# jacobswan1/ViTCAP

Hardware: AMD Instinct MI355X
Metric: images/sec end-to-end greedy caption (20 tok), ViT-B/16-384 (higher is better)
Workload: dtype bf16; 1 GPU; BASELINE configs[1]: ViT-B/16-384 greedy decode (20 tok), batch 64 bf16 per GPU, seeded random-init weights, uniform(-1,1) 384x384 images resident in HBM; batch_per_gpu=64, global_batch=64, decode=greedy, max_length=20, parallelism=replicas x1 (no data-path collective), launch=2-slot batch pipeline (encode of step i+1 || decode of step i), eager launches, streams_per_gpu=2

## Files before the change

### vitcap_amd/csrc/gemm.hip

```cpp
#include <stdio.h>
#include <stdlib.h>

#include "common.h"
#include "gemm_args.h"


#include <algorithm>
#include <mutex>
#include <utility>
#include <vector>

namespace {

int tile_group_n(int tiles_n) {
  return tiles_n > 9 ? 3 : tiles_n;
}

}
int vc_tile_group_n(int tiles_n) { return tile_group_n(tiles_n); }
namespace {

__device__ __forceinline__ void glds16(const void* g, void* lds) {
  __builtin_amdgcn_global_load_lds((const __attribute__((address_space(1))) void*)g,
                                   (__attribute__((address_space(3))) void*)lds, 16, 0, 0);
// ... 215 lines not shown
      const u32x2_t t = __builtin_amdgcn_permlane32_swap(r[c][k], r[c + 2][k], false, false);
      r[c][k] = t[0];
      r[c + 2][k] = t[1];
    }
#pragma unroll
  for (int c = 0; c < 4; c += 2)
#pragma unroll
    for (int k = 0; k < NREG; ++k) {
      const u32x2_t t = __builtin_amdgcn_permlane16_swap(r[c][k], r[c + 1][k], false, false);
      r[c][k] = t[0];
      r[c + 1][k] = t[1];
    }
}

template <int ACT, int OUT_F32, bool HAS_RES, int NI>
__device__ __forceinline__ void epilogue_direct(f32x4 (&acc)[NI][4], const GemmArgs& p, int row0, int col0, int lane) {
  const int frow = lane & 15, fk = lane >> 4;
  f32x4 bias4[4];
#pragma unroll
  for (int j = 0; j < 4; ++j) {
    const int n = col0 + j * 16 + fk * 4;
    bias4[j] = (p.bias && n < p.N) ? *(const f32x4*)(p.bias + n) : f32x4{0.f, 0.f, 0.f, 0.f};
  }
  const int ncol = col0 + fk * 16;
  const bool col_ok = ncol < p.N;
  f32x4 rres[2][4];
#define ISSUE_RES_D(i_)                                                                                    \
  if (HAS_RES) {                                                                                           \
    const int m_ = row0 + (i_) * 16 + frow;                                                                \
    _Pragma("unroll") for (int q = 0; q < 4; ++q)                                                          \
      rres[(i_) & 1][q] = (m_ < p.M && col_ok) ? *(const f32x4*)(p.res + (size_t)m_ * p.ldr + ncol + q * 4) \
                                               : f32x4{0.f, 0.f, 0.f, 0.f};                                \
  }
  ISSUE_RES_D(0);
#pragma unroll
  for (int i = 0; i < NI; ++i) {
    if (i + 1 < NI) { ISSUE_RES_D(i + 1); }
    const int m = row0 + i * 16 + frow;
    f32x4 v[4];
#pragma unroll
    for (int j = 0; j < 4; ++j) {
      v[j] = acc[i][j] + bias4[j];
      if (ACT == VITCAP_ACT_GELU_ERF) {
        v[j] = gelu_erf4(v[j]);
      }
    }
    if (OUT_F32) {
      unsigned r[4][4];
#pragma unroll
      for (int j = 0; j < 4; ++j)
#pragma unroll
        for (int e = 0; e < 4; ++e) r[j][e] = __float_as_uint(v[j][e]);
      lane_tile_transpose<4>(r);
      if (m < p.M && col_ok) {
        float* dst = (float*)p.C + (size_t)m * p.ldc + ncol;
#pragma unroll
        for (int q = 0; q < 4; ++q) {
          f32x4 o = f32x4{__uint_as_float(r[q][0]), __uint_as_float(r[q][1]), __uint_as_float(r[q][2]), __uint_as_float(r[q][3])};
          if (HAS_RES) o += rres[i & 1][q];
          *(f32x4*)(dst + q * 4) = o;
        }
      }
    } else {
      unsigned r[4][2];
#pragma unroll
      for (int j = 0; j < 4; ++j) {
        r[j][0] = pack2bf(v[j][0], v[j][1]);
        r[j][1] = pack2bf(v[j][2], v[j][3]);
      }
      lane_tile_transpose<2>(r);
      if (m < p.M && col_ok) {
        bf16_t* dst = (bf16_t*)p.C + (size_t)m * p.ldc + ncol;
        uint4 o0, o1;
        o0.x = r[0][0]; o0.y = r[0][1]; o0.z = r[1][0]; o0.w = r[1][1];
        o1.x = r[2][0]; o1.y = r[2][1]; o1.z = r[3][0]; o1.w = r[3][1];
        *(uint4*)dst = o0;
        *(uint4*)(dst + 8) = o1;
      }
    }
  }
#undef ISSUE_RES_D
}

template <int ACT, int OUT_F32, bool HAS_RES, int PH, int MT>
__device__ __forceinline__ void gemm256_tile(const GemmArgs& p, char* smem, const int m0, const int n0, const int cidx = 0) {
  constexpr int BK = 64;
  constexpr int A_BYTES = 256 * BK * 2, BUF_BYTES = 2 * A_BYTES;
  constexpr int WR = 32 * MT;
  constexpr int NI = 2 * MT;
  constexpr int NP = MT + 4;
  constexpr bool EXTRAS = (PH & 8) != 0;
  constexpr bool LN = (PH & 512) != 0;

  const int tid = threadIdx.x;
  const int lane = tid & 63;
  const int w = __builtin_amdgcn_readfirstlane(tid >> 6);
  const int grp = w >> 2;
  const int wm = w >> 2, wn = w & 3;

  const int srow = lane >> 3;
  const int schunk = (lane & 7) ^ (srow & 7);
  const bf16_t* aptr[MT];
  const bf16_t* wptr[4];
#pragma unroll
  for (int i = 0; i < MT; ++i) {
    int r = m0 + w * (8 * MT) + i * 8 + srow;
    r = r < p.M ? r : p.M - 1;
    aptr[i] = p.A + (size_t)r * p.lda + schunk * 8;
  }
#pragma unroll
  for (int i = 0; i < 4; ++i) {
    int c = n0 + w * 32 + i * 8 + srow;
    c = c < p.N ? c : p.N - 1;
    wptr[i] = p.W + (size_t)c * p.ldw + schunk * 8;
  }
#define STAGE_PIECES(q0_, q1_, buf_, k0_)                                                                          \
  _Pragma("unroll") for (int q = (q0_); q < (q1_); ++q) {                                                          \
    if (q < MT)                                                                                                    \
      glds16(aptr[q < MT ? q : 0] + (k0_), smem + (buf_) * BUF_BYTES + (w * (8 * MT) + q * 8) * 128);              \
    else                                                                                                           \
      glds16(wptr[q < MT ? 0 : q - MT] + (k0_), smem + (buf_) * BUF_BYTES + A_BYTES + (w * 32 + (q - MT) * 8) * 128); \
  }
#define STAGE_SLOT(s_, buf_, k0_) STAGE_PIECES(2 * (s_), (2 * (s_) + 2 < NP ? 2 * (s_) + 2 : NP), buf_, k0_)

  f32x4 acc[NI][4];
#pragma unroll
  for (int i = 0; i < NI; ++i)
#pragma unroll
    for (int j = 0; j < 4; ++j) acc[i][j] = f32x4{0.f, 0.f, 0.f, 0.f};

  const int frow = lane & 15;
  const int fk = lane >> 4;
  const int coff0 = ((0 * 4 + fk) ^ (frow & 7)) * 16;
  const int coff1 = ((1 * 4 + fk) ^ (frow & 7)) * 16;
  const int a_base = (wm * WR + frow) * 128;
  const int b_base = A_BYTES + (wn * 64 + frow) * 128;
  const int nk = p.K / BK;

  bf16x8 afr[MT][2];
  bf16x8 bfr[2][2][2];

#define LOAD_A(buf_, mh_)                                                                        \
  _Pragma("unroll") for (int mt = 0; mt < MT; ++mt) {                                            \
    const char* ra_ = smem + (buf_) * BUF_BYTES + a_base + ((mh_) * MT + mt) * 16 * 128;         \
    afr[mt][0] = *(const bf16x8*)(ra_ + coff0);                                                  \
    afr[mt][1] = *(const bf16x8*)(ra_ + coff1);                                                  \
  }
#define LOAD_B(buf_, nh_)                                                                        \
  _Pragma("unroll") for (int nt = 0; nt < 2; ++nt) {                                             \
    const char* rb_ = smem + (buf_) * BUF_BYTES + b_base + ((nh_) * 2 + nt) * 16 * 128;          \
    bfr[nh_][nt][0] = *(const bf16x8*)(rb_ + coff0);                                             \
    bfr[nh_][nt][1] = *(const bf16x8*)(rb_ + coff1);                                             \
  }
#define END_LOAD()                                          \
  asm volatile("s_waitcnt lgkmcnt(0)" ::: "memory");        \
  __builtin_amdgcn_sched_barrier(0);                        \
  __builtin_amdgcn_s_barrier()
#define COMPUTE(mh_, nh_)                                                                               \
  __builtin_amdgcn_s_setprio(1);                                                                        \
  _Pragma("unroll") for (int ks = 0; ks < 2; ++ks)                                                      \
    _Pragma("unroll") for (int mt = 0; mt < MT; ++mt)                                                   \
      _Pragma("unroll") for (int nt = 0; nt < 2; ++nt)                                                  \
        acc[(mh_) * MT + mt][(nh_) * 2 + nt] = __builtin_amdgcn_mfma_f32_16x16x32_bf16(                 \
            bfr[nh_][nt][ks], afr[mt][ks], acc[(mh_) * MT + mt][(nh_) * 2 + nt], 0, 0, 0);              \
  __builtin_amdgcn_s_setprio(0)

  STAGE_PIECES(0, NP, 0, 0);
  if (nk > 1) {
    STAGE_SLOT(0, 1, BK);
    asm volatile("s_waitcnt vmcnt(2)" ::: "memory");
  } else {
    asm volatile("s_waitcnt vmcnt(0)" ::: "memory");
  }
  __builtin_amdgcn_s_barrier();
  if (grp == 1) __builtin_amdgcn_s_barrier();

  for (int t = 0; t < nk; ++t) {
    const int buf = t & 1;
    const bool more = t + 1 < nk;
    const bool more2 = t + 2 < nk;
    LOAD_A(buf, 0);
    LOAD_B(buf, 0);
    if (more) { STAGE_SLOT(1, buf ^ 1, (t + 1) * BK); }
    END_LOAD();
    COMPUTE(0, 0);
    __builtin_amdgcn_s_barrier();
    LOAD_B(buf, 1);
    if (more) { STAGE_SLOT(2, buf ^ 1, (t + 1) * BK); }
    END_LOAD();
    COMPUTE(0, 1);
    __builtin_amdgcn_s_barrier();
    LOAD_A(buf, 1);
    if (more) { STAGE_SLOT(3, buf ^ 1, (t + 1) * BK); }
    END_LOAD();
    COMPUTE(1, 1);
    __builtin_amdgcn_s_barrier();
    if (more2) { STAGE_SLOT(0, buf, (t + 2) * BK); }
    if (grp == 1) {
      if (more2) asm volatile("s_waitcnt vmcnt(2)" ::: "memory");
      else asm volatile("s_waitcnt vmcnt(0)" ::: "memory");
    }
    __builtin_amdgcn_s_barrier();
    COMPUTE(1, 0);
    if (grp == 0) {
      if (more2) asm volatile("s_waitcnt vmcnt(2)" ::: "memory");
      else asm volatile("s_waitcnt vmcnt(0)" ::: "memory");
    }
    __builtin_amdgcn_s_barrier();
  }
  if (grp == 0) __builtin_amdgcn_s_barrier();
#undef STAGE_PIECES
#undef STAGE_SLOT
#undef LOAD_A
#undef LOAD_B
#undef END_LOAD
#undef COMPUTE

  constexpr int EP_ROWB = 272;
  char* ep = smem + w * (64 * EP_ROWB);
  const int er = lane >> 4, ec = (lane & 15) * 4;
  const int ncol = n0 + wn * 64 + ec;
  f32x4 bias4 = f32x4{0.f, 0.f, 0.f, 0.f};
  if (p.bias && ncol < p.N) bias4 = *(const f32x4*)(p.bias + ncol);
  const bool col_ok = ncol < p.N;
  f32x4 rres[2][2 * MT];
#define ROWS_OF(m_, orow_, rrow_)                                             \
  int orow_ = (m_), rrow_ = (m_);                                             \
  if (p.row_group > 0) {                                                      \
    const int g_ = (m_) / p.row_group, in_ = (m_) - g_ * p.row_group;         \
    orow_ = g_ * p.out_group_rows + p.out_row_off + in_;                      \
    rrow_ = p.res_periodic ? in_ : orow_;                                     \
  }
#define ISSUE_RES(c_)                                                                                        \
  if (HAS_RES) {                                                                                             \
    _Pragma("unroll") for (int it = 0; it < 2 * MT; ++it) {                                                  \
      const int m_ = m0 + wm * WR + (c_) * (8 * MT) + it * 4 + er;                                           \
      ROWS_OF(m_, o_, r_);                                                                                   \
      (void)o_;                                                                                              \
      rres[(c_) & 1][it] = (m_ < p.M && col_ok) ? *(const f32x4*)(p.res + (size_t)r_ * p.ldr + ncol)        \
                                                : f32x4{0.f, 0.f, 0.f, 0.f};                                 \
    }                                                                                                        \
  }
  if (ACT == VITCAP_ACT_GELU_ERF && !OUT_F32 && !HAS_RES && !(EXTRAS && p.zout) && !(EXTRAS && p.aux) && p.row_group == 0 &&
      (p.N & 15) == 0 && (p.ldc & 7) == 0) {
    epilogue_direct<ACT, OUT_F32, HAS_RES, NI>(acc, p, m0 + wm * WR, n0 + wn * 64, lane);
    return;
  }
  if constexpr (!OUT_F32 && !HAS_RES) {
    if (p.row_group == 0 && (p.N & 7) == 0 && (p.ldc & 7) == 0 && (!(EXTRAS && p.zout) || (p.ldz & 7) == 0) && (!(EXTRAS && p.aux) || (p.ldaux & 7) == 0)) {
      const int wr = lane >> 3, wc = (lane & 7) * 8;
      const int ncw = n0 + wn * 64 + wc;
      const bool okc = ncw < p.N;
      f32x4 b_lo = f32x4{0.f, 0.f, 0.f, 0.f}, b_hi = b_lo;
      f32x4 cs_lo = f32x4{0.f, 0.f, 0.f, 0.f}, cs_hi = cs_lo;
      if (p.bias && ncw < p.N) {
        b_lo = *(const f32x4*)(p.bias + ncw);
        b_hi = *(const f32x4*)(p.bias + ncw + 4);
      }
#pragma unroll
      for (int hm = 0; hm < 2; ++hm) {
        uint4 axv[2 * MT];
        if (EXTRAS && p.aux) {
#pragma unroll
          for (int it = 0; it < 2 * MT; ++it) {
            const int m = m0 + wm * WR + hm * (16 * MT) + it * 8 + wr;
            axv[it] = (m < p.M && okc) ? *(const uint4*)(p.aux + (size_t)m * p.ldaux + ncw) : uint4{0u, 0u, 0u, 0u};
          }
        }
#pragma unroll
        for (int i = 0; i < MT; ++i)
#pragma unroll
          for (int j = 0; j < 4; ++j)
            *(f32x4*)(ep + (i * 16 + frow) * EP_ROWB + (j * 16 + fk * 4) * 4) = acc[hm * MT + i][j];
#pragma unroll
        for (int it = 0; it < 2 * MT; ++it) {
          const int rl = it * 8 + wr;
          f32x4 v0 = *(const f32x4*)(ep + rl * EP_ROWB + wc * 4);
          f32x4 v1 = *(const f32x4*)(ep + rl * EP_ROWB + wc * 4 + 16);
          const int m = m0 + wm * WR + hm * (16 * MT) + rl;
          const bool ok = m < p.M && okc;
          v0 += b_lo;
          v1 += b_hi;
          if (EXTRAS && p.aux) {
            const uint4 a = axv[it];
            v0 *= f32x4{__uint_as_float(a.x << 16), __uint_as_float(a.x & 0xffff0000u), __uint_as_float(a.y << 16),
                        __uint_as_float(a.y & 0xffff0000u)};
            v1 *= f32x4{__uint_as_float(a.z << 16), __uint_as_float(a.z & 0xffff0000u), __uint_as_float(a.w << 16),
                        __uint_as_float(a.w & 0xffff0000u)};
          }
          if (ACT == VITCAP_ACT_GELU_ERF) {
            if (EXTRAS && p.zout) {
              f32x4 d0, d1;
              v0 = gelu_erf4_grad(v0, d0);
              v1 = gelu_erf4_grad(v1, d1);
              if (ok) {
                uint4 zo;
                zo.x = pack2bf(d0[0], d0[1]);
                zo.y = pack2bf(d0[2], d0[3]);
                zo.z = pack2bf(d1[0], d1[1]);
                zo.w = pack2bf(d1[2], d1[3]);
                *(uint4*)(p.zout + (size_t)m * p.ldz + ncw) = zo;
              }
            } else {
              v0 = gelu_erf4(v0);
              v1 = gelu_erf4(v1);
            }
          }
          if (ok) {
            uint4 o;
            o.x = pack2bf(v0[0], v0[1]);
            o.y = pack2bf(v0[2], v0[3]);
            o.z = pack2bf(v1[0], v1[1]);
            o.w = pack2bf(v1[2], v1[3]);
            *(uint4*)((bf16_t*)p.C + (size_t)m * p.ldc + ncw) = o;
            if (EXTRAS && p.colsum) {
              cs_lo += f32x4{__uint_as_float(o.x << 16), __uint_as_float(o.x & 0xffff0000u), __uint_as_float(o.y << 16),
                             __uint_as_float(o.y & 0xffff0000u)};
              cs_hi += f32x4{__uint_as_float(o.z << 16), __uint_as_float(o.z & 0xffff0000u), __uint_as_float(o.w << 16),
                             __uint_as_float(o.w & 0xffff0000u)};
            }
          }
        }
      }
      if (EXTRAS && p.colsum) {
#pragma unroll
        for (int e = 0; e < 4; ++e) {
#pragma unroll
          for (int o = 8; o <= 32; o <<= 1) {
            cs_lo[e] += __shfl_xor(cs_lo[e], o, 64);
            cs_hi[e] += __shfl_xor(cs_hi[e], o, 64);
          }
        }
        if (wr == 0 && okc) {
#pragma unroll
          for (int e = 0; e < 4; ++e) {
            atomicAdd(p.colsum + ncw + e, cs_lo[e]);
            atomicAdd(p.colsum + ncw + 4 + e, cs_hi[e]);
          }
        }
      }
      return;
    }
  }
  const __amdgpu_buffer_rsrc_t ln_rc = vc_rsrc(LN ? (const char*)p.C + (size_t)m0 * p.ldc * 4 : nullptr, LN ? (long long)(p.M - m0) * p.ldc * 4 : 0);
  ISSUE_RES(0);
#pragma unroll
  for (int hm = 0; hm < 2; ++hm) {
#pragma unroll
    for (int i = 0; i < MT; ++i)
#pragma unroll
      for (int j = 0; j < 4; ++j)
        *(f32x4*)(ep + (i * 16 + frow) * EP_ROWB + (j * 16 + fk * 4) * 4) = acc[hm * MT + i][j];
#pragma unroll
    for (int ch = 0; ch < 2; ++ch) {
      const int c = hm * 2 + ch;
      if (c + 1 < 4) { ISSUE_RES(c + 1); }
#pragma unroll
      for (int it = 0; it < 2 * MT; ++it) {
        const int rl = ch * (8 * MT) + it * 4 + er;
        f32x4 v = *(const f32x4*)(ep + rl * EP_ROWB + ec * 4);
        const int m = m0 + wm * WR + hm * (16 * MT) + rl;
        const bool ok = m < p.M && col_ok;
        ROWS_OF(m, orow, rrow);
        (void)rrow;
        v += bias4;
        if (EXTRAS && p.aux && ok) {
          const bf16x4 za = *(const bf16x4*)(p.aux + (size_t)orow * p.ldaux + ncol);
          v *= f32x4{(float)za[0], (float)za[1], (float)za[2], (float)za[3]};
        }
        if (ACT == VITCAP_ACT_GELU_ERF) {
          if (EXTRAS && p.zout) {
            f32x4 d;
            v = gelu_erf4_grad(v, d);
            if (ok) {
              uint2 zo;
              zo.x = pack2bf(d[0], d[1]);
              zo.y = pack2bf(d[2], d[3]);
              *(uint2*)(p.zout + (size_t)orow * p.ldz + ncol) = zo;
            }
          } else {
            v = gelu_erf4(v);
          }
        }
        if (HAS_RES) v += rres[c & 1][it];
        if (ok) {
          if (OUT_F32) {
            if constexpr (LN) {
              __builtin_amdgcn_raw_buffer_store_b128(__builtin_bit_cast(vc_u32x4, v), ln_rc, (unsigned)((orow - m0) * p.ldc + ncol) * 4u, 0, 16);
            } else {
              *(f32x4*)((float*)p.C + (size_t)orow * p.ldc + ncol) = v;
            }
          } else {
            uint2 o;
            o.x = pack2bf(v[0], v[1]);
            o.y = pack2bf(v[2], v[3]);
            *(uint2*)((bf16_t*)p.C + (size_t)orow * p.ldc + ncol) = o;
          }
        }
      }
    }
  }
#undef ISSUE_RES
#undef ROWS_OF
  if constexpr (LN) {
    asm volatile("s_waitcnt vmcnt(0)" ::: "memory");
    __syncthreads();
    int* s_flag = (int*)smem;
    if (tid == 0) {
      const int old = __hip_atomic_fetch_add(p.ln_cnt + cidx, 1, __ATOMIC_RELAXED, __HIP_MEMORY_SCOPE_AGENT);
      const int last = old == p.tiles_n - 1;
      if (last) __hip_atomic_store(p.ln_cnt + cidx, 0, __ATOMIC_RELAXED, __HIP_MEMORY_SCOPE_AGENT);
      *s_flag = last;
    }
    __syncthreads();
    if (*s_flag == 0) return;
    if (!p.ln_out && !p.ln_out_f) return;
    if (tid == 0) __builtin_amdgcn_fence(__ATOMIC_ACQUIRE, "agent");
    __syncthreads();
    const int rows = p.M - m0 < 64 * MT ? p.M - m0 : 64 * MT;
    constexpr int RB = 8;
    for (int r0 = w * RB; r0 < rows; r0 += 8 * RB) {
      f32x4 v[RB][3];
#pragma unroll
      for (int j = 0; j < RB; ++j)
#pragma unroll
        for (int i = 0; i < 3; ++i)
          v[j][i] = __builtin_bit_cast(f32x4, __builtin_amdgcn_raw_buffer_load_b128(ln_rc, (unsigned)((r0 + j) * p.ldc + i * 256 + lane * 4) * 4u, 0, 0));
#pragma unroll
      for (int j = 0; j < RB; ++j) {
        const int row = m0 + r0 + j;
        if (r0 + j < rows)
          ln_row(v[j], p.ln_g, p.ln_b, p.ln_eps, lane, p.ln_out ? p.ln_out + (size_t)row * D768 : nullptr,
                 p.ln_out_f ? p.ln_out_f + (size_t)row * D768 : nullptr);
      }
    }
  }
}

#ifndef VC_GEMM256_VGPRS
#define VC_GEMM256_VGPRS 224
#endif
template <int ACT, int OUT_F32, bool HAS_RES, int PH, int MTS>
__global__ __launch_bounds__(512) __attribute__((amdgpu_num_vgpr(VC_GEMM256_VGPRS))) void gemm_nt_256_kernel(GemmArgs p) {
  extern __shared__ __attribute__((aligned(16))) char smem[];
  int bid = blockIdx.x;
  const bool small = MTS != 0 && bid >= p.n_big;
  if (small) bid -= p.n_big;
  const int tiles_m = small ? p.tiles_m_small : p.tiles_m;
  {
    const int nwg = tiles_m * p.tiles_n;
    const int q = nwg >> 3, r = nwg & 7, xcd = bid & 7;
    bid = (xcd < r ? xcd * (q + 1) : r * (q + 1) + (xcd - r) * q) + (bid >> 3);
  }
  const int per_g = tiles_m * p.group_n;
  const int gi = bid / per_g, rem = bid - gi * per_g;
  const int gleft = p.tiles_n - gi * p.group_n;
  const int gw = gleft < p.group_n ? gleft : p.group_n;
  int tm = rem / gw;
  const int tn = gi * p.group_n + rem - tm * gw;
  if ((p.rev != 0) != ((gi & 1) != 0)) tm = tiles_m - 1 - tm;
  if (!small) {
    gemm256_tile<ACT, OUT_F32, HAS_RES, PH, 4>(p, smem, tm * 256, tn * 256, tm);
  } else {
    if constexpr (MTS != 0) gemm256_tile<ACT, OUT_F32, HAS_RES, PH, MTS>(p, smem, p.tiles_m * 256 + tm * (64 * MTS), tn * 256, p.tiles_m + tm);
  }
}

struct TilePlan { int tm_big, mts, tm_small; };
TilePlan plan_tiles(int M, int tiles_n, int K) {
  static const int n_cu = [] {
    int dev = 0;
    hipDeviceProp_t prop;
    if (hipGetDevice(&dev) == hipSuccess && hipGetDeviceProperties(&prop, dev) == hipSuccess && prop.multiProcessorCount > 0)
      return prop.multiProcessorCount;
    return 256;
  }();
  const int tm_full = (M + 255) / 256;
  TilePlan best{tm_full, 0, 0};
  struct Key { int M, tn, K; };
  static std::mutex mu;
  static std::vector<std::pair<Key, TilePlan>> cache;
  {
    std::lock_guard<std::mutex> g(mu);
    for (const auto& e : cache)
      if (e.first.M == M && e.first.tn == tiles_n && e.first.K == K) return e.second;
  }
  const float c3 = 0.80f, c2 = 0.60f;
  float best_t = ceilf((float)(tm_full * tiles_n) / n_cu);
  const float need = best_t * 0.97f;
  const int span = (int)(2.5f * n_cu / tiles_n) + 2;
  std::vector<float> heap;
  for (int mts = 3; mts >= 2; --mts) {
    const float cs = mts == 3 ? c3 : c2;
    for (int tb = tm_full - 1; tb >= 0 && tb >= tm_full - span; --tb) {
      const int rows_left = M - tb * 256;
      const int ts = (rows_left + 64 * mts - 1) / (64 * mts);
      const int nb = tb * tiles_n, ns = ts * tiles_n;
      heap.assign(n_cu, 0.f);
      for (int j = 0; j < n_cu; ++j) heap[j] = -(float)(nb / n_cu + (j < nb % n_cu ? 1 : 0));
      std::make_heap(heap.begin(), heap.end());
      float end = nb ? (float)((nb + n_cu - 1) / n_cu) : 0.f;
      for (int i = 0; i < ns; ++i) {
        std::pop_heap(heap.begin(), heap.end());
        const float f = -heap.back() + cs;
        heap.back() = -f;
        std::push_heap(heap.begin(), heap.end());
        end = f > end ? f : end;
      }
      if (end < need && end < best_t - 1e-4f) { best_t = end; best = TilePlan{tb, mts, ts}; }
    }
  }
  std::lock_guard<std::mutex> g(mu);
  cache.push_back({Key{M, tiles_n, K}, best});
  return best;
}

template <int ACT, int OUT_F32, bool HAS_RES, int PH, int MTS>
int launch_256_t(const GemmArgs& p, int nwg, hipStream_t s) {
  constexpr int smem = 8 * 64 * 272;
  auto kern = gemm_nt_256_kernel<ACT, OUT_F32, HAS_RES, PH, MTS>;
  VC_FUNC_SMEM(kern, smem);
  VC_LAUNCH_GEMM(kern, dim3(nwg), dim3(512), smem, s, p);
  VC_LAUNCH_CHECK("gemm_nt_256");
  return VITCAP_OK;
}

template <int ACT, int OUT_F32, bool HAS_RES, int PH>
int launch_256(const GemmArgs& a, hipStream_t s, int mix = 0) {
  if constexpr ((PH & 512) != 0) mix = 0;
  GemmArgs p = a;
  p.tiles_n = (a.N + 255) / 256;
  p.group_n = tile_group_n(p.tiles_n);
  TilePlan pl{(a.M + 255) / 256, 0, 0};
  if (a.aux || a.zout || a.colsum) mix = 0;
  if (mix < 0) pl = plan_tiles(a.M, p.tiles_n, a.K);
  else if (mix > 0) pl = TilePlan{0, mix, (a.M + 64 * mix - 1) / (64 * mix)};
  p.tiles_m = pl.tm_big;
  p.tiles_m_small = pl.tm_small;
  p.n_big = pl.tm_big * p.tiles_n;
  const int nwg = p.n_big + pl.tm_small * p.tiles_n;
  if constexpr ((PH & 512) == 0) {
    if (a.aux || a.zout || a.colsum) return launch_256_t<ACT, OUT_F32, HAS_RES, PH | 8, 0>(p, nwg, s);
    if (pl.mts == 3) return launch_256_t<ACT, OUT_F32, HAS_RES, PH, 3>(p, nwg, s);
    if (pl.mts == 2) return launch_256_t<ACT, OUT_F32, HAS_RES, PH, 2>(p, nwg, s);
  }
  return launch_256_t<ACT, OUT_F32, HAS_RES, PH, 0>(p, nwg, s);
}

template <int PH>
int dispatch_256(const GemmArgs& a, int act, int out_f32, hipStream_t s, int mix = 0) {
  const bool res = a.res != nullptr;
#define CASE(ACT_, OUT_)                                                  \
  if (act == ACT_ && out_f32 == OUT_)                                     \
    return res ? launch_256<ACT_, OUT_, true, PH>(a, s, mix) : launch_256<ACT_, OUT_, false, PH>(a, s, mix);
  CASE(VITCAP_ACT_NONE, 0)
  CASE(VITCAP_ACT_NONE, 1)
  CASE(VITCAP_ACT_GELU_ERF, 0)
  CASE(VITCAP_ACT_GELU_ERF, 1)
#undef CASE
  vitcap_set_error("gemm(256): unsupported act %d / out %d", act, out_f32);
  return VITCAP_EINVAL;
}


struct SkinnyArgs {
  GemmArgs g;
  int split_k;
  int kc;
  size_t slab;
};

template <int WAVES_M, int ACT, int OUT_F32, bool HAS_RES, bool PARTIAL>
__global__ __launch_bounds__(256) void gemm_skinny_kernel(SkinnyArgs q) {
  constexpr int WAVES_N = 4 / WAVES_M;
  constexpr int BM = 32 * WAVES_M, BN = 32 * WAVES_N;
  const GemmArgs& p = q.g;
  VC_LIVE_EXIT(p.live);
  const int lane = threadIdx.x & 63;
  const int w = __builtin_amdgcn_readfirstlane(threadIdx.x >> 6);
  const int wm = w / WAVES_N, wn = w % WAVES_N;
  const int n0 = blockIdx.x * BN + wn * 32;
  const int m0 = blockIdx.y * BM + wm * 32;
  const int kz = blockIdx.z;
  const int kbeg = kz * q.kc;
  const int frow = lane & 15, fk = lane >> 4;

  const bf16_t* ap[2];
  const bf16_t* wp[2];
#pragma unroll
  for (int i = 0; i < 2; ++i) {
    int r = m0 + i * 16 + frow;
    r = r < p.M ? r : p.M - 1;
    ap[i] = p.A + (size_t)r * p.lda + kbeg + fk * 8;
    int c = n0 + i * 16 + frow;
    c = c < p.N ? c : p.N - 1;
    wp[i] = p.W + (size_t)c * p.ldw + kbeg + fk * 8;
  }
  f32x4 acc[2][2];
#pragma unroll
  for (int i = 0; i < 2; ++i)
#pragma unroll
    for (int j = 0; j < 2; ++j) acc[i][j] = f32x4{0.f, 0.f, 0.f, 0.f};

  bf16x8 a0[4][2], w0[4][2], a1[4][2], w1[4][2];
#define LOADSET(A_, W_, k0_)                                                   \
  _Pragma("unroll") for (int s_ = 0; s_ < 4; ++s_) {                           \
    _Pragma("unroll") for (int i_ = 0; i_ < 2; ++i_) {                         \
      A_[s_][i_] = *(const bf16x8*)(ap[i_] + (k0_) + s_ * 32);                 \
      W_[s_][i_] = *(const bf16x8*)(wp[i_] + (k0_) + s_ * 32);                 \
    }                                                                          \
  }
#define MMASET(A_, W_)                                                                          \
  _Pragma("unroll") for (int s_ = 0; s_ < 4; ++s_)                                              \
    _Pragma("unroll") for (int i_ = 0; i_ < 2; ++i_)                                            \
      _Pragma("unroll") for (int j_ = 0; j_ < 2; ++j_)                                          \
        acc[i_][j_] = __builtin_amdgcn_mfma_f32_16x16x32_bf16(W_[s_][j_], A_[s_][i_], acc[i_][j_], 0, 0, 0);

  const int nch = q.kc / 128;
  LOADSET(a0, w0, 0);
  for (int c = 0; c < nch; c += 2) {
    if (c + 1 < nch) { LOADSET(a1, w1, (c + 1) * 128); }
    MMASET(a0, w0);
    if (c + 1 < nch) {
      if (c + 2 < nch) { LOADSET(a0, w0, (c + 2) * 128); }
      MMASET(a1, w1);
    }
  }
// ... 76 lines not shown
  hipLaunchKernelGGL(kern, dim3(p.tiles_m * p.tiles_n, a.split_k > 1 ? a.split_k : 1), dim3(256), smem, s, p);
  VC_LAUNCH_CHECK("gemm_nt");
  return VITCAP_OK;
}

template <int WM, int WN, int ACT, int OUT_F32, bool HAS_RES>
int launch_resident(const GemmArgs& a, hipStream_t s) {
  constexpr int BM = 32 * WM, BN = 32 * WN, NST = 12;
  constexpr int smem = NST * (BM + BN) * 64 * 2;
  static_assert(smem <= 160 * 1024, "resident tile does not fit the LDS");
  auto kern = gemm_nt_kernel<WM, WN, ACT, OUT_F32, HAS_RES, NST>;
  VC_FUNC_SMEM(kern, smem);
  GemmArgs p = a;
  p.tiles_m = (a.M + BM - 1) / BM;
  p.tiles_n = (a.N + BN - 1) / BN;
  const int splits = a.K / 768;
  if (splits > 1) {
    p.split_k = splits;
    p.kt_per_split = 12;
    p.slab = (size_t)a.M * a.ldc;
  }
  hipLaunchKernelGGL(kern, dim3(p.tiles_m * p.tiles_n, splits), dim3(256), smem, s, p);
  VC_LAUNCH_CHECK("gemm_nt(resident)");
  return VITCAP_OK;
}

template <int WM, int WN>
int dispatch_resident(const GemmArgs& a, int act, int out_f32, hipStream_t s) {
  const bool res = a.res != nullptr;
  if (a.K > 768) return launch_resident<WM, WN, VITCAP_ACT_NONE, 1, false>(a, s);
  if (act == VITCAP_ACT_NONE && !out_f32 && !res) return launch_resident<WM, WN, VITCAP_ACT_NONE, 0, false>(a, s);
  if (act == VITCAP_ACT_NONE && out_f32 && !res) return launch_resident<WM, WN, VITCAP_ACT_NONE, 1, false>(a, s);
  if (act == VITCAP_ACT_NONE && out_f32 && res) return launch_resident<WM, WN, VITCAP_ACT_NONE, 1, true>(a, s);
  if (act == VITCAP_ACT_GELU_ERF && !out_f32 && !res) return launch_resident<WM, WN, VITCAP_ACT_GELU_ERF, 0, false>(a, s);
  if (act == VITCAP_ACT_GELU_ERF && out_f32 && !res) return launch_resident<WM, WN, VITCAP_ACT_GELU_ERF, 1, false>(a, s);
  vitcap_set_error("gemm(resident): unsupported epilogue act=%d out=%d res=%d", act, out_f32, (int)res);
  return VITCAP_EINVAL;
}

template <int WM, int WN, int NST>
int launch_rowstat_t(const GemmArgs& a, hipStream_t s) {
  constexpr int BM = 32 * WM, BN = 32 * WN, smem = NST * (BM + BN) * 64 * 2;
  auto kern = gemm_nt_kernel<WM, WN, VITCAP_ACT_NONE, 1, false, NST, true>;
  VC_FUNC_SMEM(kern, smem);
  GemmArgs p = a;
  p.tiles_m = (a.M + BM - 1) / BM;
  p.tiles_n = (a.N + BN - 1) / BN;
  hipLaunchKernelGGL(kern, dim3(p.tiles_m * p.tiles_n, 1), dim3(256), smem, s, p);
  VC_LAUNCH_CHECK("gemm_nt(rowstat)");
  return VITCAP_OK;
}

int launch_rowstat(const GemmArgs& a, hipStream_t s) {
  return a.M <= 256 ? launch_rowstat_t<2, 2, 4>(a, s) : launch_rowstat_t<4, 4, 2>(a, s);
}

template <int WM, int WN>
int dispatch(const GemmArgs& a, int act, int out_f32, hipStream_t s) {
  const bool res = a.res != nullptr;
#define CASE(ACT_, OUT_)                                                         \
  if (act == ACT_ && out_f32 == OUT_)                                            \
    return res ? launch<WM, WN, ACT_, OUT_, true>(a, s) : launch<WM, WN, ACT_, OUT_, false>(a, s);
  CASE(VITCAP_ACT_NONE, 0)
  CASE(VITCAP_ACT_NONE, 1)
  CASE(VITCAP_ACT_GELU_ERF, 0)
  CASE(VITCAP_ACT_GELU_ERF, 1)
  CASE(VITCAP_ACT_TANH, 0)
  CASE(VITCAP_ACT_TANH, 1)
#undef CASE
  vitcap_set_error("gemm: unsupported act %d / out %d", act, out_f32);
  return VITCAP_EINVAL;
}

}

static int large_gemm_form(int M, int hint, bool plain_bf16) {
  if (M < 2048) return -1;
  if (hint == 0) return 2;
  if (hint == 5) return plain_bf16 && M < 65536 ? 1 : -1;
  return -1;
}

static bool known_tile_hint(int h) {
  return h == 0 || h == 1 || h == 2 || h == 4 || h == 5 || (h >= 13 && h <= 15) || (h >= 20 && h <= 24) || (h >= 30 && h <= 33) ||
         (h >= 40 && h <= 42);
}

extern "C" int vitcap_gemm_large_form(int M, int N, int K, int tile_hint) {
  const bool plain_bf16 = (tile_hint & 0x100) != 0;
  tile_hint &= 0xff;
  int form = large_gemm_form(M, tile_hint, plain_bf16);
  if (form < 0) return -1;
  if (K < 128) return -1;
  if (form == 2 && (K < 192 || (N & 255) != 0)) form = 1;
  if (form != 0 && (N & 7) != 0) form = 0;
  return form + 10 * vc_4w_pick_mi(M, (N + 255) / 256, form);
}

extern "C" int vitcap_gemm_ex(const void* A, const void* W, const float* bias, const float* residual, void* C,
                              const vitcap_gemm_desc* d, const void* aux_bf16, int ldaux, void* zout_bf16, int ldz,
                              void* stream);

extern "C" int vitcap_gemm_tile_plan(int M, int N, int K, int* plan3) {
  VC_REQUIRE(M > 0 && N > 0 && K > 0 && plan3, "gemm_tile_plan: bad arguments");
  const TilePlan pl = plan_tiles(M, (N + 255) / 256, K);
  plan3[0] = pl.tm_big;
  plan3[1] = pl.mts;
  plan3[2] = pl.tm_small;
  return VITCAP_OK;
}

extern "C" int vitcap_gemm_bias_act(const void* A, const void* W, const float* bias, const float* residual,
                                    void* C, const vitcap_gemm_desc* d, void* stream) {
  return vitcap_gemm_ex(A, W, bias, residual, C, d, nullptr, 0, nullptr, 0, stream);
}

extern "C" int vitcap_gemm_ex(const void* A, const void* W, const float* bias, const float* residual, void* C,
                              const vitcap_gemm_desc* d, const void* aux_bf16, int ldaux, void* zout_bf16, int ldz,
                              void* stream) {
  VC_REQUIRE(A && W && C && d, "gemm: null pointer");
  VC_REQUIRE(d->abi == VITCAP_ABI_VERSION, "gemm: descriptor built against ABI %d, this library is ABI %d", d->abi, VITCAP_ABI_VERSION);
  VC_REQUIRE(d->M > 0 && d->N > 0 && d->K > 0, "gemm: empty problem M=%d N=%d K=%d", d->M, d->N, d->K);
  VC_REQUIRE(d->K % 64 == 0, "gemm: K=%d must be a multiple of 64", d->K);
  VC_REQUIRE(d->N % 4 == 0 && d->ldc % 4 == 0, "gemm: N=%d and ldc=%d must be multiples of 4", d->N, d->ldc);
  VC_REQUIRE(d->lda % 8 == 0 && d->ldw % 8 == 0, "gemm: lda=%d ldw=%d must be multiples of 8", d->lda, d->ldw);
  VC_REQUIRE(((uintptr_t)A & 15) == 0 && ((uintptr_t)W & 15) == 0 && ((uintptr_t)C & 15) == 0,
             "gemm: A/W/C must be 16-byte aligned");
  VC_REQUIRE(!residual || (d->ldr % 4 == 0 && ((uintptr_t)residual & 15) == 0), "gemm: residual misaligned");
  VC_REQUIRE(!bias || ((uintptr_t)bias & 15) == 0, "gemm: bias misaligned");
  GemmArgs a;
  a.A = (const bf16_t*)A;
  a.W = (const bf16_t*)W;
  a.bias = bias;
  a.res = residual;
  a.C = C;
  a.M = d->M; a.N = d->N; a.K = d->K;
  a.lda = d->lda; a.ldw = d->ldw; a.ldc = d->ldc; a.ldr = d->ldr;
  a.row_group = d->row_group; a.out_group_rows = d->out_group_rows;
  a.out_row_off = d->out_row_off; a.res_periodic = d->res_periodic;
  a.tiles_m = a.tiles_n = 0;
  a.aux = (const bf16_t*)aux_bf16; a.ldaux = ldaux;
  a.colsum = d->colsum;
  a.zout = (bf16_t*)zout_bf16; a.ldz = ldz;
  a.split_k = 1; a.kt_per_split = 0; a.slab = 0;
  a.live = d->live;
  a.rev = vc_tls_walk_rev ? 1 : 0;
  a.rowstat = (float*)d->rowstat;
  a.ln_g = a.ln_b = nullptr; a.ln_eps = 0.f; a.ln_out = nullptr; a.ln_out_f = nullptr; a.ln_cnt = nullptr;
  VC_REQUIRE(!(aux_bf16 && d->act != VITCAP_ACT_NONE), "gemm: aux (gelu') epilogue needs act == none");
  VC_REQUIRE(!zout_bf16 || d->act == VITCAP_ACT_GELU_ERF, "gemm: zout stores the GELU's derivative and needs act == gelu_erf");
  VC_REQUIRE(known_tile_hint(d->tile_hint), "gemm: unknown tile_hint %d", d->tile_hint);
  hipStream_t s = (hipStream_t)stream;
  const int hint = d->tile_hint;
  const int split_k = d->split_k > 1 ? d->split_k : 1;
  const bool plain_rows = d->row_group == 0;
  if (d->ln_out_bf16 || d->ln_out_f32) {
    VC_REQUIRE(d->ln_gamma && d->ln_beta, "gemm(ln): ln_gamma / ln_beta missing");
    VC_REQUIRE(d->N == 768 && d->ldc == 768 && d->out_dtype == VITCAP_OUT_F32 && d->act == VITCAP_ACT_NONE && plain_rows && split_k == 1 &&
                   !aux_bf16 && !zout_bf16 && !d->rowstat && !d->colsum,
               "gemm(ln): needs N == ldc == 768, fp32 output, no activation / row remap / split-K / training extras");
    const bool fused = d->ln_counters && d->M >= 2048 && hint == 5;
    if (fused) {
      a.ln_g = d->ln_gamma; a.ln_b = d->ln_beta; a.ln_eps = d->ln_eps;
      a.ln_out = (bf16_t*)d->ln_out_bf16; a.ln_out_f = d->ln_out_f32; a.ln_cnt = d->ln_counters;
      return residual ? launch_256<VITCAP_ACT_NONE, 1, true, 4 | 512>(a, s, 0) : launch_256<VITCAP_ACT_NONE, 1, false, 4 | 512>(a, s, 0);
    }
    vitcap_gemm_desc d2 = *d;
    d2.ln_out_bf16 = nullptr; d2.ln_out_f32 = nullptr;
    const int rc = vitcap_gemm_ex(A, W, bias, residual, C, &d2, aux_bf16, ldaux, zout_bf16, ldz, stream);
    if (rc != VITCAP_OK) return rc;
    const bool dir = vc_tls_walk_rev;
    if (vc_tls_zigzag && d->M >= 2048) vc_tls_walk_rev = !dir;
    const int rc2 = vitcap_layernorm_fwd((const float*)C, d->ldc, d->ln_gamma, d->ln_beta, d->ln_eps, d->ln_out_bf16, d->ln_out_f32, d->M, 768, stream);
    vc_tls_walk_rev = dir;
    return rc2;
  }
  if (d->rowstat) {
    VC_REQUIRE(d->out_dtype == VITCAP_OUT_F32 && d->act == VITCAP_ACT_NONE && !residual && plain_rows && split_k == 1 && !aux_bf16 && !zout_bf16,
               "gemm(rowstat): fp32 output, no activation / residual / split-K");
    return launch_rowstat(a, s);
  }
  if (d->colsum) {
    VC_REQUIRE(d->out_dtype == VITCAP_OUT_BF16 && !residual && plain_rows && split_k == 1 && d->M >= 2048 && d->N % 8 == 0 && d->ldc % 8 == 0 &&
                   (!aux_bf16 || ldaux % 8 == 0) && (!zout_bf16 || ldz % 8 == 0) && d->act != VITCAP_ACT_TANH,
               "gemm(colsum): needs bf16 output, no residual / row remap / split-K, M >= 2048, N, ldc (ldaux, ldz) multiples of 8");
    if (hint == 42 && vc_4w_supports(a, d->act))
      return vc_dispatch_4w(a, d->act, d->out_dtype, s, 2);
    return dispatch_256<4>(a, d->act, d->out_dtype, s, 0);
  }
  if (hint == 23 || hint == 24) {
    VC_REQUIRE(d->K % 768 == 0 && d->K > 768 && plain_rows && !aux_bf16 && !zout_bf16 && d->out_dtype == VITCAP_OUT_F32 && !bias && !residual &&
                   d->act == VITCAP_ACT_NONE,
               "gemm(ring slabs): needs K a multiple of 768 above it, plain rows, raw fp32 slabs (no bias / residual / activation)");
    a.split_k = d->K / 768;
    a.kt_per_split = 12;
    a.slab = (size_t)d->M * d->ldc;
    return hint == 23 ? dispatch<2, 1>(a, VITCAP_ACT_NONE, 1, s) : dispatch<1, 1>(a, VITCAP_ACT_NONE, 1, s);
  }
  if (hint == 20 || hint == 21 || hint == 22) {
    VC_REQUIRE(d->K % 768 == 0 && plain_rows && !aux_bf16 && !zout_bf16, "gemm(resident): needs K %% 768 == 0, plain rows, no training extras");
    VC_REQUIRE(d->K == 768 || (d->out_dtype == VITCAP_OUT_F32 && !bias && !residual && d->act == VITCAP_ACT_NONE),
               "gemm(resident): K > 768 writes raw fp32 partial slabs");
    if (hint == 20) return dispatch_resident<2, 1>(a, d->act, d->out_dtype, s);
    if (hint == 21) return dispatch_resident<1, 1>(a, d->act, d->out_dtype, s);
    return dispatch_resident<1, 2>(a, d->act, d->out_dtype, s);
  }
  if (split_k > 1 && d->M > 256) {
    VC_REQUIRE(d->out_dtype == VITCAP_OUT_F32 && plain_rows && !aux_bf16 && !zout_bf16, "gemm: split-K writes fp32 partial slabs only");
    const int nk = d->K / 64;
    a.split_k = split_k;
    a.kt_per_split = (nk + split_k - 1) / split_k;
    a.slab = (size_t)d->M * d->ldc;
    return dispatch<4, 4>(a, VITCAP_ACT_NONE, 1, s);
  }
  if (split_k > 1) {
    VC_REQUIRE(d->K % (128 * split_k) == 0, "gemm: K=%d not divisible into %d splits of multiples of 128", d->K, split_k);
    VC_REQUIRE(d->out_dtype == VITCAP_OUT_F32 && plain_rows, "gemm: split-K writes fp32 partial slabs only");
  }
  if (split_k > 1 || hint == 4) {
    VC_REQUIRE(d->K % 128 == 0 && plain_rows, "gemm(skinny): needs K %% 128 == 0 and no row remap");
    return d->M <= 64 ? launch_skinny<2>(a, d->act, d->out_dtype, split_k, s)
                      : launch_skinny<4>(a, d->act, d->out_dtype, split_k, s);
  }
  if (hint == 13) return dispatch<2, 1>(a, d->act, d->out_dtype, s);
  if (hint == 14) return dispatch<1, 1>(a, d->act, d->out_dtype, s);
  if (hint == 15) return dispatch<1, 2>(a, d->act, d->out_dtype, s);
  if (hint == 0 && d->M <= 128) return dispatch<1, 1>(a, d->act, d->out_dtype, s);
  if (hint == 1 || (hint == 0 && d->M <= 256)) return dispatch<2, 2>(a, d->act, d->out_dtype, s);
  if (hint == 0 && d->act != VITCAP_ACT_TANH) {
    const float kf = d->K > 768 ? (float)(d->K - 768) / 2304.f : 0.f;
    const auto grid = [&](int t) { return (float)(((d->M + t - 1) / t) * ((d->N + t - 1) / t)); };
    const float t64 = 4.f + grid(64) * (0.0165f + kf * 0.0385f);
    const float t128 = fmaxf(16.f + kf * 26.f, 9.f + grid(128) * (0.0375f + kf * 0.0745f));
    const float t256 = d->M >= 2048 ? ceilf(grid(256) / 256.f) * (23.f + kf * 57.f) : 1e30f;
    if (t64 < t128 && t64 < t256) return dispatch<2, 2>(a, d->act, d->out_dtype, s);
    if (t128 < t256) return dispatch<4, 4>(a, d->act, d->out_dtype, s);
  }
  if (hint == 2 || (hint == 0 && (d->M < 2048 || d->act == VITCAP_ACT_TANH)))
    return dispatch<4, 4>(a, d->act, d->out_dtype, s);
  if (hint >= 40 && hint <= 42) {
    VC_REQUIRE(!(aux_bf16 || zout_bf16 || d->colsum) || (hint == 42 && d->out_dtype == VITCAP_OUT_BF16),
               "gemm(4-wave): aux / zout / colsum need the persistent form (tile_hint 42) and a bf16 output");
    return vc_dispatch_4w(a, d->act, d->out_dtype, s, hint - 40);
  }
  if (hint == 30) return dispatch_256<4>(a, d->act, d->out_dtype, s, 3);
  if (hint == 31) return dispatch_256<4>(a, d->act, d->out_dtype, s, 2);
  if (hint == 32) return dispatch_256<4>(a, d->act, d->out_dtype, s, 0);
  if (hint == 33) return dispatch_256<4>(a, d->act, d->out_dtype, s, -1);
  const int form = large_gemm_form(d->M, hint, !(d->out_dtype == VITCAP_OUT_F32 || residual));
  if (form >= 0 && !(aux_bf16 || zout_bf16 || d->colsum) && vc_4w_supports(a, d->act)) return vc_dispatch_4w(a, d->act, d->out_dtype, s, form);
  return dispatch_256<4>(a, d->act, d->out_dtype, s, hint == 5 ? 0 : -1);
}
```

Baseline: 4021 images/sec.

## Generalize 256-wide GEMM tile to 16-row granularity and pick uniform tile height

The 256-tile GEMM kernel is re-parameterized by the number of 16-row MFMA slices (NI) instead of 32-row pairs, so uneven tile heights such as 224 or 192 rows are possible. Waves in the two groups stage different A-row counts and the epilogue masks the missing slices. A new uniform planner (used for hint 5 instead of the fixed 256 tile) picks 256, 224 or 192-row tiles from a wave-count cost model to reduce tail waves on the CU count. The trade-off is extra branching, uneven per-wave work and more template instantiations.

```diff
diff --git a/vitcap_amd/csrc/gemm.hip b/vitcap_amd/csrc/gemm.hip
--- a/vitcap_amd/csrc/gemm.hip
+++ b/vitcap_amd/csrc/gemm.hip
@@ -321,13 +321,12 @@
 #undef ISSUE_RES_D
 }
 
-template <int ACT, int OUT_F32, bool HAS_RES, int PH, int MT>
+template <int ACT, int OUT_F32, bool HAS_RES, int PH, int NI>
 __device__ __forceinline__ void gemm256_tile(const GemmArgs& p, char* smem, const int m0, const int n0, const int cidx = 0) {
   constexpr int BK = 64;
   constexpr int A_BYTES = 256 * BK * 2, BUF_BYTES = 2 * A_BYTES;
-  constexpr int WR = 32 * MT;
-  constexpr int NI = 2 * MT;
-  constexpr int NP = MT + 4;
+  constexpr int WR = 16 * NI;
+  constexpr int MH0 = (NI + 1) / 2, MH1 = NI / 2;
   constexpr bool EXTRAS = (PH & 8) != 0;
   constexpr bool LN = (PH & 512) != 0;
 
@@ -339,11 +338,12 @@
 
   const int srow = lane >> 3;
   const int schunk = (lane & 7) ^ (srow & 7);
-  const bf16_t* aptr[MT];
+  const int arow0 = (MH0 == MH1 || w < 4 ? w * MH0 : 4 * MH0 + (w - 4) * MH1) * 8;
+  const bf16_t* aptr[MH0];
   const bf16_t* wptr[4];
 #pragma unroll
-  for (int i = 0; i < MT; ++i) {
-    int r = m0 + w * (8 * MT) + i * 8 + srow;
+  for (int i = 0; i < MH0; ++i) {
+    int r = m0 + arow0 + i * 8 + srow;
     r = r < p.M ? r : p.M - 1;
     aptr[i] = p.A + (size_t)r * p.lda + schunk * 8;
   }
@@ -353,14 +353,17 @@
     c = c < p.N ? c : p.N - 1;
     wptr[i] = p.W + (size_t)c * p.ldw + schunk * 8;
   }
-#define STAGE_PIECES(q0_, q1_, buf_, k0_)                                                                          \
-  _Pragma("unroll") for (int q = (q0_); q < (q1_); ++q) {                                                          \
-    if (q < MT)                                                                                                    \
-      glds16(aptr[q < MT ? q : 0] + (k0_), smem + (buf_) * BUF_BYTES + (w * (8 * MT) + q * 8) * 128);              \
+#define STAGE_PIECES_N(na_, q0_, q1_, buf_, k0_)                                                                   \
+  _Pragma("unroll") for (int q = (q0_); q < ((q1_) < (na_) + 4 ? (q1_) : (na_) + 4); ++q) {                        \
+    if (q < (na_))                                                                                                 \
+      glds16(aptr[q < (na_) ? q : 0] + (k0_), smem + (buf_) * BUF_BYTES + (arow0 + q * 8) * 128);                  \
     else                                                                                                           \
-      glds16(wptr[q < MT ? 0 : q - MT] + (k0_), smem + (buf_) * BUF_BYTES + A_BYTES + (w * 32 + (q - MT) * 8) * 128); \
-  }
-#define STAGE_SLOT(s_, buf_, k0_) STAGE_PIECES(2 * (s_), (2 * (s_) + 2 < NP ? 2 * (s_) + 2 : NP), buf_, k0_)
+      glds16(wptr[q < (na_) ? 0 : q - (na_)] + (k0_), smem + (buf_) * BUF_BYTES + A_BYTES + (w * 32 + (q - (na_)) * 8) * 128); \
+  }
+#define STAGE_PIECES(q0_, q1_, buf_, k0_)                                   \
+  if (MH0 == MH1 || grp == 0) { STAGE_PIECES_N(MH0, q0_, q1_, buf_, k0_); } \
+  else { STAGE_PIECES_N(MH1, q0_, q1_, buf_, k0_); }
+#define STAGE_SLOT(s_, buf_, k0_) STAGE_PIECES(2 * (s_), 2 * (s_) + 2, buf_, k0_)
 
   f32x4 acc[NI][4];
 #pragma unroll
@@ -376,12 +379,12 @@
   const int b_base = A_BYTES + (wn * 64 + frow) * 128;
   const int nk = p.K / BK;
 
-  bf16x8 afr[MT][2];
+  bf16x8 afr[MH0][2];
   bf16x8 bfr[2][2][2];
 
 #define LOAD_A(buf_, mh_)                                                                        \
-  _Pragma("unroll") for (int mt = 0; mt < MT; ++mt) {                                            \
-    const char* ra_ = smem + (buf_) * BUF_BYTES + a_base + ((mh_) * MT + mt) * 16 * 128;         \
+  _Pragma("unroll") for (int mt = 0; mt < ((mh_) ? MH1 : MH0); ++mt) {                           \
+    const char* ra_ = smem + (buf_) * BUF_BYTES + a_base + ((mh_) * MH0 + mt) * 16 * 128;        \
     afr[mt][0] = *(const bf16x8*)(ra_ + coff0);                                                  \
     afr[mt][1] = *(const bf16x8*)(ra_ + coff1);                                                  \
   }
@@ -398,13 +401,13 @@
 #define COMPUTE(mh_, nh_)                                                                               \
   __builtin_amdgcn_s_setprio(1);                                                                        \
   _Pragma("unroll") for (int ks = 0; ks < 2; ++ks)                                                      \
-    _Pragma("unroll") for (int mt = 0; mt < MT; ++mt)                                                   \
+    _Pragma("unroll") for (int mt = 0; mt < ((mh_) ? MH1 : MH0); ++mt)                                  \
       _Pragma("unroll") for (int nt = 0; nt < 2; ++nt)                                                  \
-        acc[(mh_) * MT + mt][(nh_) * 2 + nt] = __builtin_amdgcn_mfma_f32_16x16x32_bf16(                 \
-            bfr[nh_][nt][ks], afr[mt][ks], acc[(mh_) * MT + mt][(nh_) * 2 + nt], 0, 0, 0);              \
+        acc[(mh_) * MH0 + mt][(nh_) * 2 + nt] = __builtin_amdgcn_mfma_f32_16x16x32_bf16(                \
+            bfr[nh_][nt][ks], afr[mt][ks], acc[(mh_) * MH0 + mt][(nh_) * 2 + nt], 0, 0, 0);             \
   __builtin_amdgcn_s_setprio(0)
 
-  STAGE_PIECES(0, NP, 0, 0);
+  STAGE_PIECES(0, 8, 0, 0);
   if (nk > 1) {
     STAGE_SLOT(0, 1, BK);
     asm volatile("s_waitcnt vmcnt(2)" ::: "memory");
@@ -448,6 +451,7 @@
     __builtin_amdgcn_s_barrier();
   }
   if (grp == 0) __builtin_amdgcn_s_barrier();
+#undef STAGE_PIECES_N
 #undef STAGE_PIECES
 #undef STAGE_SLOT
 #undef LOAD_A
@@ -462,7 +466,7 @@
   f32x4 bias4 = f32x4{0.f, 0.f, 0.f, 0.f};
   if (p.bias && ncol < p.N) bias4 = *(const f32x4*)(p.bias + ncol);
   const bool col_ok = ncol < p.N;
-  f32x4 rres[2][2 * MT];
+  f32x4 rres[2][2 * MH0];
 #define ROWS_OF(m_, orow_, rrow_)                                             \
   int orow_ = (m_), rrow_ = (m_);                                             \
   if (p.row_group > 0) {                                                      \
@@ -472,12 +476,14 @@
   }
 #define ISSUE_RES(c_)                                                                                        \
   if (HAS_RES) {                                                                                             \
-    _Pragma("unroll") for (int it = 0; it < 2 * MT; ++it) {                                                  \
-      const int m_ = m0 + wm * WR + (c_) * (8 * MT) + it * 4 + er;                                           \
+    _Pragma("unroll") for (int it = 0; it < 2 * MH0; ++it) {                                                 \
+      const int mh_ = (c_) >> 1 ? MH1 : MH0;                                                                 \
+      const int m_ = m0 + wm * WR + ((c_) >> 1) * (16 * MH0) + ((c_) & 1) * (8 * mh_) + it * 4 + er;         \
       ROWS_OF(m_, o_, r_);                                                                                   \
       (void)o_;                                                                                              \
-      rres[(c_) & 1][it] = (m_ < p.M && col_ok) ? *(const f32x4*)(p.res + (size_t)r_ * p.ldr + ncol)        \
-                                                : f32x4{0.f, 0.f, 0.f, 0.f};                                 \
+      if (it < 2 * mh_)                                                                                      \
+        rres[(c_) & 1][it] = (m_ < p.M && col_ok) ? *(const f32x4*)(p.res + (size_t)r_ * p.ldr + ncol)      \
+                                                  : f32x4{0.f, 0.f, 0.f, 0.f};                               \
     }                                                                                                        \
   }
   if (ACT == VITCAP_ACT_GELU_ERF && !OUT_F32 && !HAS_RES && !(EXTRAS && p.zout) && !(EXTRAS && p.aux) && p.row_group == 0 &&
@@ -498,25 +504,27 @@
       }
 #pragma unroll
       for (int hm = 0; hm < 2; ++hm) {
-        uint4 axv[2 * MT];
+        const int mh = hm ? MH1 : MH0;
+        uint4 axv[2 * MH0];
         if (EXTRAS && p.aux) {
 #pragma unroll
-          for (int it = 0; it < 2 * MT; ++it) {
-            const int m = m0 + wm * WR + hm * (16 * MT) + it * 8 + wr;
-            axv[it] = (m < p.M && okc) ? *(const uint4*)(p.aux + (size_t)m * p.ldaux + ncw) : uint4{0u, 0u, 0u, 0u};
+          for (int it = 0; it < 2 * MH0; ++it) {
+            const int m = m0 + wm * WR + hm * (16 * MH0) + it * 8 + wr;
+            if (it < 2 * mh) axv[it] = (m < p.M && okc) ? *(const uint4*)(p.aux + (size_t)m * p.ldaux + ncw) : uint4{0u, 0u, 0u, 0u};
           }
         }
 #pragma unroll
-        for (int i = 0; i < MT; ++i)
+        for (int i = 0; i < MH0; ++i)
 #pragma unroll
           for (int j = 0; j < 4; ++j)
-            *(f32x4*)(ep + (i * 16 + frow) * EP_ROWB + (j * 16 + fk * 4) * 4) = acc[hm * MT + i][j];
-#pragma unroll
-        for (int it = 0; it < 2 * MT; ++it) {
+            if (i < mh) *(f32x4*)(ep + (i * 16 + frow) * EP_ROWB + (j * 16 + fk * 4) * 4) = acc[hm * MH0 + (i < mh ? i : 0)][j];
+#pragma unroll
+        for (int it = 0; it < 2 * MH0; ++it) {
+          if (it >= 2 * mh) continue;
           const int rl = it * 8 + wr;
           f32x4 v0 = *(const f32x4*)(ep + rl * EP_ROWB + wc * 4);
           f32x4 v1 = *(const f32x4*)(ep + rl * EP_ROWB + wc * 4 + 16);
-          const int m = m0 + wm * WR + hm * (16 * MT) + rl;
+          const int m = m0 + wm * WR + hm * (16 * MH0) + rl;
           const bool ok = m < p.M && okc;
           v0 += b_lo;
           v1 += b_hi;
@@ -585,20 +593,22 @@
   ISSUE_RES(0);
 #pragma unroll
   for (int hm = 0; hm < 2; ++hm) {
-#pragma unroll
-    for (int i = 0; i < MT; ++i)
+    const int mh = hm ? MH1 : MH0;
+#pragma unroll
+    for (int i = 0; i < MH0; ++i)
 #pragma unroll
       for (int j = 0; j < 4; ++j)
-        *(f32x4*)(ep + (i * 16 + frow) * EP_ROWB + (j * 16 + fk * 4) * 4) = acc[hm * MT + i][j];
+        if (i < mh) *(f32x4*)(ep + (i * 16 + frow) * EP_ROWB + (j * 16 + fk * 4) * 4) = acc[hm * MH0 + (i < mh ? i : 0)][j];
 #pragma unroll
     for (int ch = 0; ch < 2; ++ch) {
       const int c = hm * 2 + ch;
       if (c + 1 < 4) { ISSUE_RES(c + 1); }
 #pragma unroll
-      for (int it = 0; it < 2 * MT; ++it) {
-        const int rl = ch * (8 * MT) + it * 4 + er;
+      for (int it = 0; it < 2 * MH0; ++it) {
+        if (it >= 2 * mh) continue;
+        const int rl = ch * (8 * mh) + it * 4 + er;
         f32x4 v = *(const f32x4*)(ep + rl * EP_ROWB + ec * 4);
-        const int m = m0 + wm * WR + hm * (16 * MT) + rl;
+        const int m = m0 + wm * WR + hm * (16 * MH0) + rl;
         const bool ok = m < p.M && col_ok;
         ROWS_OF(m, orow, rrow);
         (void)rrow;
@@ -656,7 +666,7 @@
     if (!p.ln_out && !p.ln_out_f) return;
     if (tid == 0) __builtin_amdgcn_fence(__ATOMIC_ACQUIRE, "agent");
     __syncthreads();
-    const int rows = p.M - m0 < 64 * MT ? p.M - m0 : 64 * MT;
+    const int rows = p.M - m0 < 32 * NI ? p.M - m0 : 32 * NI;
     constexpr int RB = 8;
     for (int r0 = w * RB; r0 < rows; r0 += 8 * RB) {
       f32x4 v[RB][3];
@@ -679,11 +689,11 @@
 #ifndef VC_GEMM256_VGPRS
 #define VC_GEMM256_VGPRS 224
 #endif
-template <int ACT, int OUT_F32, bool HAS_RES, int PH, int MTS>
+template <int ACT, int OUT_F32, bool HAS_RES, int PH, int NIS>
 __global__ __launch_bounds__(512) __attribute__((amdgpu_num_vgpr(VC_GEMM256_VGPRS))) void gemm_nt_256_kernel(GemmArgs p) {
   extern __shared__ __attribute__((aligned(16))) char smem[];
   int bid = blockIdx.x;
-  const bool small = MTS != 0 && bid >= p.n_big;
+  const bool small = NIS != 0 && bid >= p.n_big;
   if (small) bid -= p.n_big;
   const int tiles_m = small ? p.tiles_m_small : p.tiles_m;
   {
@@ -699,14 +709,14 @@
   const int tn = gi * p.group_n + rem - tm * gw;
   if ((p.rev != 0) != ((gi & 1) != 0)) tm = tiles_m - 1 - tm;
   if (!small) {
-    gemm256_tile<ACT, OUT_F32, HAS_RES, PH, 4>(p, smem, tm * 256, tn * 256, tm);
+    gemm256_tile<ACT, OUT_F32, HAS_RES, PH, 8>(p, smem, tm * 256, tn * 256, tm);
   } else {
-    if constexpr (MTS != 0) gemm256_tile<ACT, OUT_F32, HAS_RES, PH, MTS>(p, smem, p.tiles_m * 256 + tm * (64 * MTS), tn * 256, p.tiles_m + tm);
+    if constexpr (NIS != 0) gemm256_tile<ACT, OUT_F32, HAS_RES, PH, NIS>(p, smem, p.tiles_m * 256 + tm * (32 * NIS), tn * 256, p.tiles_m + tm);
   }
 }
 
 struct TilePlan { int tm_big, mts, tm_small; };
-TilePlan plan_tiles(int M, int tiles_n, int K) {
+static int plan_n_cu() {
   static const int n_cu = [] {
     int dev = 0;
     hipDeviceProp_t prop;
@@ -714,6 +724,10 @@
       return prop.multiProcessorCount;
     return 256;
   }();
+  return n_cu;
+}
+TilePlan plan_tiles(int M, int tiles_n, int K) {
+  const int n_cu = plan_n_cu();
   const int tm_full = (M + 255) / 256;
   TilePlan best{tm_full, 0, 0};
   struct Key { int M, tn, K; };
@@ -754,10 +768,24 @@
   return best;
 }
 
-template <int ACT, int OUT_F32, bool HAS_RES, int PH, int MTS>
+#ifndef VC_TILE224_COST
+#define VC_TILE224_COST 0.90f
+#endif
+int plan_uniform(int M, int tiles_n) {
+  const int n_cu = plan_n_cu();
+  const auto cost = [&](int ni, float c) { return ceilf((float)(((M + 32 * ni - 1) / (32 * ni)) * tiles_n) / n_cu) * c; };
+  const float t8 = cost(8, 1.f), t7 = cost(7, VC_TILE224_COST), t6 = cost(6, 0.80f);
+  int ni = 8;
+  float best = t8 * 0.97f;
+  if (t7 < best) { best = t7; ni = 7; }
+  if (t6 < best) { best = t6; ni = 6; }
+  return ni;
+}
+
+template <int ACT, int OUT_F32, bool HAS_RES, int PH, int NIS>
 int launch_256_t(const GemmArgs& p, int nwg, hipStream_t s) {
   constexpr int smem = 8 * 64 * 272;
-  auto kern = gemm_nt_256_kernel<ACT, OUT_F32, HAS_RES, PH, MTS>;
+  auto kern = gemm_nt_256_kernel<ACT, OUT_F32, HAS_RES, PH, NIS>;
   VC_FUNC_SMEM(kern, smem);
   VC_LAUNCH_GEMM(kern, dim3(nwg), dim3(512), smem, s, p);
   VC_LAUNCH_CHECK("gemm_nt_256");
@@ -772,16 +800,19 @@
   p.group_n = tile_group_n(p.tiles_n);
   TilePlan pl{(a.M + 255) / 256, 0, 0};
   if (a.aux || a.zout || a.colsum) mix = 0;
-  if (mix < 0) pl = plan_tiles(a.M, p.tiles_n, a.K);
-  else if (mix > 0) pl = TilePlan{0, mix, (a.M + 64 * mix - 1) / (64 * mix)};
+  int nis = 0;
+  if (mix == -2) mix = plan_uniform(a.M, p.tiles_n) & 7;
+  if (mix == -1) { pl = plan_tiles(a.M, p.tiles_n, a.K); nis = 2 * pl.mts; }
+  else if (mix > 0) { pl = TilePlan{0, 0, (a.M + 32 * mix - 1) / (32 * mix)}; nis = mix; }
   p.tiles_m = pl.tm_big;
   p.tiles_m_small = pl.tm_small;
   p.n_big = pl.tm_big * p.tiles_n;
   const int nwg = p.n_big + pl.tm_small * p.tiles_n;
   if constexpr ((PH & 512) == 0) {
     if (a.aux || a.zout || a.colsum) return launch_256_t<ACT, OUT_F32, HAS_RES, PH | 8, 0>(p, nwg, s);
-    if (pl.mts == 3) return launch_256_t<ACT, OUT_F32, HAS_RES, PH, 3>(p, nwg, s);
-    if (pl.mts == 2) return launch_256_t<ACT, OUT_F32, HAS_RES, PH, 2>(p, nwg, s);
+    if (nis == 7) return launch_256_t<ACT, OUT_F32, HAS_RES, PH, 7>(p, nwg, s);
+    if (nis == 6) return launch_256_t<ACT, OUT_F32, HAS_RES, PH, 6>(p, nwg, s);
+    if (nis == 4) return launch_256_t<ACT, OUT_F32, HAS_RES, PH, 4>(p, nwg, s);
   }
   return launch_256_t<ACT, OUT_F32, HAS_RES, PH, 0>(p, nwg, s);
 }
@@ -1024,7 +1055,7 @@
 }
 
 static bool known_tile_hint(int h) {
-  return h == 0 || h == 1 || h == 2 || h == 4 || h == 5 || (h >= 13 && h <= 15) || (h >= 20 && h <= 24) || (h >= 30 && h <= 33) ||
+  return h == 0 || h == 1 || h == 2 || h == 4 || h == 5 || (h >= 13 && h <= 15) || (h >= 20 && h <= 24) || (h >= 30 && h <= 34) ||
          (h >= 40 && h <= 42);
 }
 
@@ -1185,11 +1216,12 @@
                "gemm(4-wave): aux / zout / colsum need the persistent form (tile_hint 42) and a bf16 output");
     return vc_dispatch_4w(a, d->act, d->out_dtype, s, hint - 40);
   }
-  if (hint == 30) return dispatch_256<4>(a, d->act, d->out_dtype, s, 3);
-  if (hint == 31) return dispatch_256<4>(a, d->act, d->out_dtype, s, 2);
+  if (hint == 30) return dispatch_256<4>(a, d->act, d->out_dtype, s, 6);
+  if (hint == 31) return dispatch_256<4>(a, d->act, d->out_dtype, s, 4);
+  if (hint == 34) return dispatch_256<4>(a, d->act, d->out_dtype, s, 7);
   if (hint == 32) return dispatch_256<4>(a, d->act, d->out_dtype, s, 0);
   if (hint == 33) return dispatch_256<4>(a, d->act, d->out_dtype, s, -1);
   const int form = large_gemm_form(d->M, hint, !(d->out_dtype == VITCAP_OUT_F32 || residual));
   if (form >= 0 && !(aux_bf16 || zout_bf16 || d->colsum) && vc_4w_supports(a, d->act)) return vc_dispatch_4w(a, d->act, d->out_dtype, s, form);
-  return dispatch_256<4>(a, d->act, d->out_dtype, s, hint == 5 ? 0 : -1);
-}
+  return dispatch_256<4>(a, d->act, d->out_dtype, s, hint == 5 ? -2 : -1);
+}
```

Measured after the change: 3976 images/sec. 0.989x the previous value.
